# shangzhouye/stereo-visual-slam

Measured on AMD Instinct MI355X. Metric: stereo keyframes/sec (ORB+match+tri+local-BA), KITTI-00 1241x376, higher is better.
Workload: dtype u8+f64

## Files before the change

### stereo-visual-slam_amd/csrc/lm_kernels.hip

```cpp
#include "vslam_internal.h"

#include <stdlib.h>

#include <vector>

#include "se3_device.h"
#include "lm_device.h"

namespace vslam {

constexpr int kLmBlock = 512;
constexpr int kLmItemFixed = 128;
constexpr int kLmMinWaves = 2;
constexpr int kLmWaves = kLmBlock / 64;
constexpr int kMaxKf = VSLAM_MAX_KF;
constexpr int kMaxNp = 6 * kMaxKf;
constexpr int kMaxPairs = kMaxKf * (kMaxKf + 1) / 2;
constexpr int kHitsPerEdge = (kMaxKf + 1) / 2 + 1;
constexpr int kDinvLds = 1950;
constexpr int kLin = 2;
constexpr int kPoseParts = 3;
constexpr int kCntStride = 80;
constexpr int kItemSlots = (kMaxPairs + kLmWaves - 1) / kLmWaves;
constexpr int kDbgSlots = 24;
// ... 1132 lines not shown
    }
    atomicAdd(&cnt, mine);
    __syncthreads();
    if (threadIdx.x == 0 && n_inl) n_inl[b] = cnt;
}

__global__ __launch_bounds__(64) void pnp_wave_kernel(const float* __restrict__ xyz, const float* __restrict__ uv, const int32_t* __restrict__ d_n, int capacity,
                                                     double* __restrict__ d_T, int iters, double K0, double K1, double K2, double K3, double delta,
                                                     double thr2, uint8_t* __restrict__ inlier, int32_t* __restrict__ n_inl, vslam_lm_stats* __restrict__ stats) {
    const int b = blockIdx.x, lane = threadIdx.x;
    const int n = min(max(d_n[b], 0), capacity);
    const float* px = xyz + 3 * (size_t)b * capacity;
    const float2* pz = reinterpret_cast<const float2*>(uv) + (size_t)b * capacity;
    const double K[4] = {K0, K1, K2, K3};
    const CamK ck = make_camk(K);
    vslam_lm_stats* st = stats ? stats + b : nullptr;
    double T[7], Rt[12];
#pragma unroll
    for (int i = 0; i < 7; ++i) T[i] = d_T[7 * (size_t)b + i];
    expand_pose(T, Rt);
    const int slot27 = wave_slot<27>(lane);
    auto evaluate = [&](const double* R, bool lin, double (&H)[36], double (&g)[6]) -> double {
        double part = 0, acc[27];
#pragma unroll
        for (int i = 0; i < 27; ++i) acc[i] = 0;
        for (int i0 = 0; i0 < n; i0 += 128) {
            const int ia = i0 + lane, ib = i0 + 64 + lane;
            const int ja = min(ia, n - 1), jb = min(ib, n - 1);
            const double ax = px[3 * ja], ay = px[3 * ja + 1], az = px[3 * ja + 2], bx = px[3 * jb], by = px[3 * jb + 1], bz = px[3 * jb + 2];
            const float2 za = pz[ja], zb = pz[jb];
#pragma unroll
            for (int u = 0; u < 2; ++u) {
                if ((u ? ib : ia) >= n) continue;
                double x, y, ri, wgt, ex, ey, c, rho;
                cam_norm(R, u ? bx : ax, u ? by : ay, u ? bz : az, x, y, ri);
                eval_obs(ck, x, y, u ? zb : za, delta, ex, ey, c, rho, wgt);
                part += rho;
                if (lin) {
                    double A[12], wA[12];
                    jac_norm(x, y, ri, A);
                    const double l0 = wgt * ck.fx2, l1 = wgt * ck.fy2;
#pragma unroll
                    for (int i = 0; i < 6; ++i) { wA[i] = l0 * A[i]; wA[6 + i] = l1 * A[6 + i]; }
                    int idx = 0;
#pragma unroll
                    for (int r = 0; r < 6; ++r)
#pragma unroll
                        for (int cc = r; cc < 6; ++cc) { acc[idx] = a_fma_pair(wA, r, A, cc, acc[idx]); ++idx; }
#pragma unroll
                    for (int r = 0; r < 6; ++r) acc[21 + r] = a_fma2(wA, r, -ex, -ey, acc[21 + r]);
                }
            }
        }
        const double total = wave_sum(part);
        if (lin) {
            wave_reduce_scatter<27>(acc, lane);
            double v[27];
#pragma unroll
            for (int sidx = 0; sidx < 27; ++sidx) {
                const int src = __ffsll((long long)__ballot(slot27 == sidx)) - 1;
                v[sidx] = readlane_f64(acc[0], src);
            }
            int idx = 0;
#pragma unroll
            for (int r = 0; r < 6; ++r)
#pragma unroll
                for (int cc = r; cc < 6; ++cc) { H[6 * r + cc] = v[idx]; H[6 * cc + r] = v[idx]; ++idx; }
#pragma unroll
            for (int r = 0; r < 6; ++r) g[r] = v[21 + r];
        }
        return total;
    };
    double H[36], g[6], lambda = 0, ni = 2, currentChi = 0;
    int it = 0, total_trials = 0;
    for (it = 0; it < iters; ++it) {
        currentChi = evaluate(Rt, true, H, g);
        if (it == 0) {
            if (st && lane == 0) st->chi2_init = currentChi;
            double md = 0;
#pragma unroll
            for (int a = 0; a < 6; ++a) md = fmax(fabs(H[7 * a]), md);
            lambda = 1e-5 * md;
            ni = 2;
        }
        double rho_gain = 0;
        int qmax = 0;
        bool again = true;
        while (again) {
            double x[6], E[7], Tt[7], Rtt[12], Hd[36], gd[6];
            const bool ok2 = chol6_solve(H, lambda, g, x);
            if (!ok2) {
#pragma unroll
                for (int i = 0; i < 6; ++i) x[i] = 0;
            }
            se3::exp(x, E);
            se3::mul(E, T, Tt);
            expand_pose(Tt, Rtt);
            double tempChi = evaluate(Rtt, false, Hd, gd);
            if (!ok2) tempChi = 1.7976931348623157e308;
            double scale = 1e-3;
#pragma unroll
            for (int i = 0; i < 6; ++i) scale += x[i] * (lambda * x[i] + g[i]);
            rho_gain = (currentChi - tempChi) / scale;
            if (rho_gain > 0 && isfinite(tempChi)) {
                double alpha = 1. - pow(2 * rho_gain - 1, 3);
                alpha = fmin(alpha, 2. / 3.);
                lambda *= fmax(1. / 3., alpha);
                ni = 2;
                currentChi = tempChi;
#pragma unroll
                for (int i = 0; i < 7; ++i) T[i] = Tt[i];
#pragma unroll
                for (int i = 0; i < 12; ++i) Rt[i] = Rtt[i];
            } else {
                lambda *= ni;
                ni *= 2;
            }
            ++qmax;
            again = (rho_gain < 0) && qmax < 10;
        }
        total_trials += qmax;
        if (st && lane == 0 && it < VSLAM_LM_MAX_ITERS) { st->chi2_iter[it] = currentChi; st->lambda_iter[it] = lambda; st->trials_iter[it] = qmax; }
        if (qmax == 10 || rho_gain == 0) { ++it; break; }
    }
    if (st && lane == 0) { st->iterations = it; st->total_trials = total_trials; st->chi2_final = currentChi; st->lambda_final = lambda; }
    if (lane < 7) d_T[7 * (size_t)b + lane] = T[lane];
    int mine = 0;
    for (int i = lane; i < n; i += 64) {
        const size_t gi = (size_t)b * capacity + i;
        double X, Y, Z, ex, ey;
        project_err(Rt, K, (double)px[3 * i], (double)px[3 * i + 1], (double)px[3 * i + 2], uv[2 * gi], uv[2 * gi + 1], X, Y, Z, ex, ey);
        const double c = ex * ex + ey * ey;
        const bool ok = isfinite(c) && c <= thr2;
        if (inlier) inlier[gi] = ok;
        mine += ok;
    }
    for (int o = 32; o > 0; o >>= 1) mine += __shfl_xor(mine, o);
    if (lane == 0 && n_inl) n_inl[b] = mine;
}

struct PoShared {
    double H[2][kMaxKf][36], g[2][kMaxKf][6];
    double part[2][kMaxKf], spart[2][kMaxKf];
    double x[kMaxKf][6];
    int cnt[kMaxKf][kMaxKf];
    int kbeg[kMaxKf + 1];
    int flag[2];
    int cin[2][kMaxKf], cout[2][kMaxKf];
    double T[2][kMaxKf][7], R[3][kMaxKf][12];
};
template <int W, int kMinWaves>
__global__ __launch_bounds__(64 * W, kMinWaves) void pose_only_wave_kernel(LmKernelArgs ka, int iters, int update_poses) {
    static_assert(W == kMaxKf || (W >= 1 && W <= 8), "the keyframe deal takes its minimum over eight lanes");
    constexpr int kBlock = 64 * W;
    const LmWindowArgs& a = ka.a;
    __shared__ PoShared sm;
    const int w = ka.order ? ka.order[blockIdx.x] : (int)blockIdx.x, tid = threadIdx.x, lane = tid & 63;
    const int wave = __builtin_amdgcn_readfirstlane(tid >> 6);
    if (ka.status[w] != VSLAM_OK) return;
    long long* cyc = ka.dbg_cycles ? ka.dbg_cycles + kDbgSlots * (size_t)w : nullptr;
    long long t_ph = cyc ? clock64() : 0;
#define POH(i) do { if (cyc && tid == 0) { const long long t1__ = clock64(); cyc[i] += t1__ - t_ph; t_ph = t1__; } } while (0)
    const int nk = a.n_kf_w ? min(max(a.n_kf_w[w], 1), a.n_kf) : a.n_kf;
    const int lm0 = a.lm_off[w], e0 = a.edge_off[w], ne = a.edge_off[w + 1] - e0;
    const int32_t* kfi = a.kf_idx + e0;
    const int32_t* lmi = a.lm_idx + e0;
    const float2* uv2 = reinterpret_cast<const float2*>(a.uv) + e0;
    const float* xyz = a.xyz + 3 * (size_t)lm0;
    uint8_t* inl = a.lm_inlier + lm0;
    int32_t* list = a.kf_edges + e0;
    float2* uvk = reinterpret_cast<float2*>(ka.uvk) + e0;
    float4* posk = reinterpret_cast<float4*>(a.lin) + e0;
    double* chik = ka.chi2k + e0;
    const double K[4] = {a.K[0], a.K[1], a.K[2], a.K[3]};
    const CamK ck = make_camk(K);
    const double delta = a.huber_delta;
    const unsigned long long lt_mask = (1ull << lane) - 1ull;
    const int per = (((ne + W - 1) / W) + 63) & ~63;
    const int c0 = min(wave * per, ne), c1 = min(c0 + per, ne);
    {
        int cnt[kMaxKf];
#pragma unroll
        for (int k = 0; k < kMaxKf; ++k) cnt[k] = 0;
        for (int base = c0; base < c1; base += 256) {
            int kq[4], lq[4]; bool vq[4]; uint8_t iq[4];
#pragma unroll
            for (int u = 0; u < 4; ++u) { const int e = base + 64 * u + lane; vq[u] = e < c1; const int es = min(e, ne - 1); kq[u] = kfi[es]; lq[u] = lmi[es]; }
#pragma unroll
            for (int u = 0; u < 4; ++u) iq[u] = inl[lq[u]];
#pragma unroll
            for (int u = 0; u < 4; ++u) {
                const bool act = vq[u] && iq[u] != 0;
#pragma unroll
                for (int kk = 0; kk < kMaxKf; ++kk) cnt[kk] += __popcll(__ballot(act && kq[u] == kk));
            }
        }
        if (lane < kMaxKf) {
            int v = 0;
#pragma unroll
            for (int kk = 0; kk < kMaxKf; ++kk) if (lane == kk) v = cnt[kk];
            sm.cnt[wave][lane] = v;
        }
        if (tid < 2) sm.flag[tid] = 0;
    }
    __syncthreads();
    int off[kMaxKf];
    {
        int run = 0;
#pragma unroll
        for (int k = 0; k < kMaxKf; ++k) {
            int before = 0, tot = 0;
#pragma unroll
            for (int c = 0; c < W; ++c) { const int v = sm.cnt[c][k]; tot += v; if (c < wave) before += v; }
            off[k] = run + before;
            if (tid == 0) sm.kbeg[k] = run;
            run += tot;
        }
        if (tid == 0) sm.kbeg[kMaxKf] = run;
    }
    for (int base = c0; base < c1; base += 256) {
        int kq[4], lq[4], eq[4]; bool vq[4]; uint8_t iq[4]; float2 zq[4]; float Xq[4], Yq[4], Zq[4];
#pragma unroll
        for (int u = 0; u < 4; ++u) {
            const int e = base + 64 * u + lane; vq[u] = e < c1; eq[u] = e;
            const int es = min(e, ne - 1);
            kq[u] = kfi[es]; lq[u] = lmi[es]; zq[u] = uv2[es];
        }
#pragma unroll
        for (int u = 0; u < 4; ++u) { iq[u] = inl[lq[u]]; Xq[u] = xyz[3 * lq[u]]; Yq[u] = xyz[3 * lq[u] + 1]; Zq[u] = xyz[3 * lq[u] + 2]; }
#pragma unroll
        for (int u = 0; u < 4; ++u) {
            const bool act = vq[u] && iq[u] != 0;
#pragma unroll
            for (int kk = 0; kk < kMaxKf; ++kk) {
                const unsigned long long m = __ballot(act && kq[u] == kk);
                if (act && kq[u] == kk) {
                    const int pos = off[kk] + __popcll(m & lt_mask);
                    list[pos] = eq[u]; uvk[pos] = zq[u]; posk[pos] = make_float4(Xq[u], Yq[u], Zq[u], 0.f);
                }
                off[kk] += __popcll(m);
            }
        }
    }
    __syncthreads();
    POH(0);
    unsigned long long held = 0;
    int nheld = 0;
    if constexpr (W == kMaxKf) { held = (unsigned long long)wave; nheld = wave < nk ? 1 : 0; }
    else {
        const int kl = min(lane, kMaxKf - 1);
        const int mycnt = lane < nk ? sm.kbeg[kl + 1] - sm.kbeg[kl] : -1;
        int rank = 0;
        for (int j = 0; j < nk; ++j) { const int cj = sm.kbeg[j + 1] - sm.kbeg[j]; rank += (cj > mycnt || (cj == mycnt && j < lane)) ? 1 : 0; }
        int load = 0;
        for (int r = 0; r < nk; ++r) {
            const int k = __builtin_amdgcn_readfirstlane(__ffsll((long long)__ballot(lane < nk && rank == r)) - 1);
            const int cr = __shfl(mycnt, k);
            int key = lane < W ? load * 16 + lane : 0x7fffffff;
            key = min(key, __shfl_xor(key, 1)); key = min(key, __shfl_xor(key, 2)); key = min(key, __shfl_xor(key, 4));
            const int v = __builtin_amdgcn_readfirstlane(key) & 15;
            if (lane == v) load += cr;
            if (v == wave) { held |= (unsigned long long)k << (4 * nheld); ++nheld; }
        }
    }
    auto kf_at = [&](int q) -> int { return (int)((held >> (4 * q)) & 15ull); };
#pragma unroll 1
    for (int q = 0; q < nheld; ++q) {
        const int k = kf_at(q);
        double T[7], Rt[12];
#pragma unroll
        for (int i = 0; i < 7; ++i) T[i] = a.T[((size_t)w * a.n_kf + k) * 7 + i];
        expand_pose(T, Rt);
        if (lane == 0) {
#pragma unroll
            for (int i = 0; i < 7; ++i) sm.T[0][k][i] = T[i];
#pragma unroll
            for (int i = 0; i < 12; ++i) { sm.R[0][k][i] = Rt[i]; sm.R[2][k][i] = Rt[i]; }
        }
    }
    __builtin_amdgcn_wave_barrier();
    const int slot27 = wave_slot<27>(lane);
    auto evaluate = [&](const double* Rlds, bool lin, int buf, bool store_chi, int k) -> double {
        const int kb = __builtin_amdgcn_readfirstlane(sm.kbeg[k]), ke = __builtin_amdgcn_readfirstlane(sm.kbeg[k + 1]);
        double R[12];
#pragma unroll
        for (int i = 0; i < 12; ++i) R[i] = uniform_f64(Rlds[i]);
        double part = 0, acc[27];
#pragma unroll
        for (int i = 0; i < 27; ++i) acc[i] = 0;
        float4 pp[2], pn[2]; float2 zz[2], zn[2];
#pragma unroll
        for (int u = 0; u < 2; ++u) { const int j = min(kb + 64 * u + lane, max(ke - 1, 0)); pp[u] = posk[j]; zz[u] = uvk[j]; }
        for (int j0 = kb; j0 < ke; j0 += 128) {
#pragma unroll
            for (int u = 0; u < 2; ++u) { const int j = min(j0 + 128 + 64 * u + lane, ke - 1); pn[u] = posk[j]; zn[u] = uvk[j]; }
#pragma unroll
            for (int u = 0; u < 2; ++u) {
                const int j = j0 + 64 * u + lane;
                if (j >= ke) continue;
                double x, y, ri, wgt, ex, ey, c, rho;
                cam_norm(R, (double)pp[u].x, (double)pp[u].y, (double)pp[u].z, x, y, ri);
                eval_obs(ck, x, y, zz[u], delta, ex, ey, c, rho, wgt);
                part += rho;
                if (store_chi) chik[j] = c;
                if (lin) {
                    double A[12], wA[12];
                    jac_norm(x, y, ri, A);
                    const double l0 = wgt * ck.fx2, l1 = wgt * ck.fy2;
#pragma unroll
                    for (int i = 0; i < 6; ++i) { wA[i] = l0 * A[i]; wA[6 + i] = l1 * A[6 + i]; }
                    int idx = 0;
#pragma unroll
                    for (int r = 0; r < 6; ++r)
#pragma unroll
                        for (int cc = r; cc < 6; ++cc) { acc[idx] = a_fma_pair(wA, r, A, cc, acc[idx]); ++idx; }
#pragma unroll
                    for (int r = 0; r < 6; ++r) acc[21 + r] = a_fma2(wA, r, -ex, -ey, acc[21 + r]);
                }
            }
#pragma unroll
            for (int u = 0; u < 2; ++u) { pp[u] = pn[u]; zz[u] = zn[u]; }
        }
        const double total = wave_sum(part);
        if (lin) {
            wave_reduce_scatter<27>(acc, lane);
            if (slot27 >= 0 && slot27 < 21) {
                int r = 0, rem = slot27;
                while (rem >= 6 - r) { rem -= 6 - r; ++r; }
                const int cc = r + rem;
                sm.H[buf][k][6 * r + cc] = acc[0]; sm.H[buf][k][6 * cc + r] = acc[0];
            } else if (slot27 >= 21) sm.g[buf][k][slot27 - 21] = acc[0];
        }
        return total;
    };
    auto sum_kf = [&](const double* v) -> double {
        double t = 0;
        for (int k = 0; k < nk; ++k) t += v[k];
        return t;
    };
    vslam_lm_stats* st = a.stats ? a.stats + w : nullptr;
    double lambda = 0, ni = 2, currentChi = 0;
    int pc = 0;
    int cur = 0, it = 0, total_trials = 0, pb = 0, fb = 0;
    if (iters > 0) {
#pragma unroll 1
        for (int q = 0; q < nheld; ++q) {
            const int k = kf_at(q);
            const double c = evaluate(sm.R[pc][k], true, cur, false, k);
            if (lane == 0) sm.part[pb][k] = c;
        }
        __syncthreads();
        currentChi = sum_kf(sm.part[pb]);
        pb ^= 1;
        double md = 0;
        for (int k = 0; k < nk; ++k)
#pragma unroll
            for (int d = 0; d < 6; ++d) md = fmax(md, fabs(sm.H[cur][k][7 * d]));
        lambda = 1e-5 * md;
        if (st && tid == 0) st->chi2_init = currentChi;
    }
    POH(1);
    for (it = 0; it < iters; ++it) {
        double rho_gain = 0;
        int qmax = 0;
        bool again = true;
        while (again) {
            double xw[6] = {0, 0, 0, 0, 0, 0};
#pragma unroll 1
            for (int q = 0; q < nheld; ++q) {
                const int k = kf_at(q);
                double Hk[36], gk[6], x[6] = {0, 0, 0, 0, 0, 0};
#pragma unroll
                for (int i = 0; i < 36; ++i) Hk[i] = sm.H[cur][k][i];
#pragma unroll
                for (int i = 0; i < 6; ++i) gk[i] = sm.g[cur][k][i];
                if (!chol6_solve(Hk, lambda, gk, x) && lane == 0) sm.flag[fb] = 1;
                if constexpr (W == kMaxKf) {
#pragma unroll
                    for (int i = 0; i < 6; ++i) xw[i] = x[i];
                } else if (lane == 0) {
#pragma unroll
                    for (int i = 0; i < 6; ++i) sm.x[k][i] = x[i];
                }
            }
            POH(2);
            __syncthreads();
            POH(3);
            const bool ok2 = sm.flag[fb] == 0;
            if (tid == 0) sm.flag[fb ^ 1] = 0;
            fb ^= 1;
#pragma unroll 1
            for (int q = 0; q < nheld; ++q) {
                const int k = kf_at(q);
                double sc = 0;
                {
                    double x[6], E[7], Tc[7], Tt[7], Rtt[12];
#pragma unroll
                    for (int i = 0; i < 6; ++i) x[i] = !ok2 ? 0.0 : W == kMaxKf ? xw[i] : sm.x[k][i];
#pragma unroll
                    for (int i = 0; i < 6; ++i) sc += x[i] * (lambda * x[i] + sm.g[cur][k][i]);
#pragma unroll
                    for (int i = 0; i < 7; ++i) Tc[i] = sm.T[pc][k][i];
                    se3::exp(x, E);
                    se3::mul(E, Tc, Tt);
                    expand_pose(Tt, Rtt);
                    __builtin_amdgcn_wave_barrier();
                    if (lane == 0) {
#pragma unroll
                        for (int i = 0; i < 7; ++i) sm.T[pc ^ 1][k][i] = Tt[i];
#pragma unroll
                        for (int i = 0; i < 12; ++i) { sm.R[pc ^ 1][k][i] = Rtt[i]; sm.R[2][k][i] = Rtt[i]; }
                    }
                    __builtin_amdgcn_wave_barrier();
                }
                POH(4);
                const double c = evaluate(sm.R[pc ^ 1][k], true, cur ^ 1, false, k);
                POH(5);
                if (lane == 0) { sm.part[pb][k] = c; sm.spart[pb][k] = sc; }
            }
            __syncthreads();
            POH(6);
            double tempChi = sum_kf(sm.part[pb]);
            const double scale = sum_kf(sm.spart[pb]) + 1e-3;
            pb ^= 1;
            if (!ok2) tempChi = 1.7976931348623157e308;
            rho_gain = (currentChi - tempChi) / scale;
            if (rho_gain > 0 && isfinite(tempChi)) {
                double alpha = 1. - pow(2 * rho_gain - 1, 3);
                alpha = fmin(alpha, 2. / 3.);
                lambda *= fmax(1. / 3., alpha);
                ni = 2;
                currentChi = tempChi;
                pc ^= 1;
                cur ^= 1;
            } else {
                lambda *= ni;
                ni *= 2;
            }
            ++qmax;
            again = (rho_gain < 0) && qmax < 10;
        }
        total_trials += qmax;
        if (st && tid == 0 && it < VSLAM_LM_MAX_ITERS) { st->chi2_iter[it] = currentChi; st->lambda_iter[it] = lambda; st->trials_iter[it] = qmax; }
        if (qmax == 10 || rho_gain == 0) { ++it; break; }
    }
    if (st && tid == 0) { st->iterations = it; st->total_trials = total_trials; st->chi2_final = currentChi; st->lambda_final = lambda; }
    POH(7);
#pragma unroll 1
    for (int q = 0; q < nheld; ++q) { const int k = kf_at(q); evaluate(sm.R[2][k], false, 0, true, k); }
    double th = delta;
    int cb = 0;
    for (int iteration = 0; iteration < 5; ++iteration) {
#pragma unroll 1
        for (int q = 0; q < nheld; ++q) {
            const int k = kf_at(q), kb = sm.kbeg[k], ke = sm.kbeg[k + 1];
            int cin = 0, cout = 0;
            for (int j = kb + lane; j < ke; j += 64) { if (chik[j] > th) ++cout; else ++cin; }
            for (int o = 32; o > 0; o >>= 1) { cin += __shfl_xor(cin, o); cout += __shfl_xor(cout, o); }
            if (lane == 0) { sm.cin[cb][k] = cin; sm.cout[cb][k] = cout; }
        }
        __syncthreads();
        int tin = 0, tout = 0;
        for (int k = 0; k < nk; ++k) { tin += sm.cin[cb][k]; tout += sm.cout[cb][k]; }
        cb ^= 1;
        const double ratio = (double)tin / (double)(tin + tout);
        if (ratio > 0.5) break;
        th *= 2;
    }
    if (ka.want_chi2) {
        double* chi2 = a.chi2 + e0;
        for (int e = tid; e < ne; e += kBlock) if (!inl[lmi[e]]) chi2[e] = 0.0;
#pragma unroll 1
        for (int q = 0; q < nheld; ++q) {
            const int k = kf_at(q), kb = sm.kbeg[k], ke = sm.kbeg[k + 1];
            for (int j = kb + lane; j < ke; j += 64) chi2[list[j]] = chik[j];
        }
    }
    __syncthreads();
#pragma unroll 1
    for (int q = 0; q < nheld; ++q) {
        const int k = kf_at(q), kb = sm.kbeg[k], ke = sm.kbeg[k + 1];
        for (int j = kb + lane; j < ke; j += 64) {
            const int e = list[j];
            if (e == ne - 1 || lmi[e + 1] != lmi[e]) inl[lmi[e]] = !(chik[j] > th);
        }
        if (update_poses && lane < 7) a.T[((size_t)w * a.n_kf + k) * 7 + lane] = sm.T[pc][k][lane];
    }
    if (tid == 0 && a.chi2_thr) a.chi2_thr[w] = th;
    POH(8);
#undef POH
}

static int carve_lm(LmScratch& s, LmKernelArgs& ka, size_t total_lm, size_t total_edge, int n_windows, bool with_lm, hipStream_t stream) {
    int32_t* defer;
    if (int rc = carve(s.buf, stream, [&](Layout& L) {
            ka.a.P = L.take<double>(total_lm * 3);
            ka.a.Ptrial = L.take<double>(total_lm * 3);
            ka.a.Hll = L.take<double>(total_lm * 6);
            ka.a.bl = L.take<double>(total_lm * 3);
            ka.a.Dinv = L.take<double>(total_lm * 6);
            ka.a.lin = L.take<double>(total_edge * kLin);
            ka.a.lm_ptr = L.take<int32_t>(total_lm + n_windows + 1);
            ka.a.kf_ptr = L.take<int32_t>((size_t)n_windows * (kMaxKf + 1));
            ka.a.kf_edges = L.take<int32_t>(total_edge);
            ka.a.pair_ptr = L.take<int32_t>((size_t)n_windows * (kMaxPairs + 1));
            ka.a.pair_hits = L.take<int32_t>(with_lm ? total_edge * kHitsPerEdge * 2 : 64);
            ka.act = L.take<uint8_t>(total_lm);
            ka.kf_pos = L.take<int32_t>(total_edge);
            ka.status = L.take<int32_t>(n_windows);
            double* chi2 = L.take<double>(total_edge);
            if (!ka.a.chi2) ka.a.chi2 = chi2;
            ka.chi2k = L.take<double>(total_edge);
            ka.uvk = L.take<float>(total_edge * 2);
            ka.slot_uv = L.take<float>(with_lm ? total_lm * kLmSlots * 2 : 64);
            ka.slot_kf = L.take<uint8_t>(with_lm ? total_lm * kLmSlots : 256);
            ka.lcnt = L.take<uint8_t>(total_lm);
            ka.order = L.take<int32_t>(n_windows);
            ka.passes = L.take<int32_t>(n_windows);
            defer = L.take<int32_t>(n_windows);
        })) return rc;
    s.status = ka.status; s.status_n = n_windows; s.passes = ka.passes; s.defer = defer;
    return VSLAM_OK;
}

__global__ void lm_fill_kernel(int32_t* __restrict__ p, int n, int v) { const int i = blockIdx.x * blockDim.x + threadIdx.x; if (i < n) p[i] = v; }
constexpr int kOrderCap = 4096;
__global__ __launch_bounds__(1024) void lm_order_kernel(const int32_t* __restrict__ edge_off, int n, int32_t* __restrict__ order) {
    __shared__ unsigned long long key[kOrderCap];
    int np2 = 1;
    while (np2 < n) np2 <<= 1;
    for (int i = threadIdx.x; i < np2; i += 1024)
        key[i] = i < n ? ((unsigned long long)(0xFFFFFFFFu - (unsigned)max(edge_off[i + 1] - edge_off[i], 0)) << 32) | (unsigned)i : ~0ull;
    for (int k = 2; k <= np2; k <<= 1)
        for (int j = k >> 1; j > 0; j >>= 1) {
            __syncthreads();
            for (int t = threadIdx.x; t < np2 / 2; t += 1024) {
                const int lo = ((t / j) * 2 * j) + (t % j), hi = lo + j;
                const bool up = (lo & k) == 0;
                const unsigned long long x = key[lo], y = key[hi];
                if ((x > y) == up) { key[lo] = y; key[hi] = x; }
            }
        }
    __syncthreads();
    for (int i = threadIdx.x; i < n; i += 1024) order[i] = (int32_t)(key[i] & 0xFFFFFFFFu);
}

int launch_lm_windows(const LmWindowArgs& a, int schedule, int mode, int iters, int update_poses, int update_lms, LmScratch* scratch,
                      hipStream_t stream) {
    const size_t total_lm = a.total_lm, total_edge = a.total_edge;
    if (a.n_windows <= 0) return VSLAM_OK;
    if (a.n_kf <= 0 || a.n_kf > kMaxKf) { set_error("n_kf %d out of range (1..%d)", a.n_kf, kMaxKf); return VSLAM_ERR_ARG; }
    LmKernelArgs ka;
    memset(&ka, 0, sizeof(ka));
    ka.a = a;
    ka.want_chi2 = a.chi2 != nullptr;
    ka.dinv_lds = kDinvLds;
    const size_t dyn_lds = (size_t)kDinvLds * 6 * sizeof(double);
    if (!scratch->lds_opt_in) {
        VS_HIP(hipFuncSetAttribute(reinterpret_cast<const void*>(&lm_window_kernel<false>), hipFuncAttributeMaxDynamicSharedMemorySize, (int)dyn_lds));
        VS_HIP(hipFuncSetAttribute(reinterpret_cast<const void*>(&lm_window_kernel<false, true>), hipFuncAttributeMaxDynamicSharedMemorySize, (int)dyn_lds));
        scratch->lds_opt_in = true;
    }
    if (getenv("VSLAM_LM_PROFILE")) {
        const size_t cyc_need = sizeof(long long) * kDbgSlots * a.n_windows;
        if (int rc = scratch->cyc.reserve(cyc_need, stream)) return rc;
        VS_HIP(hipMemsetAsync(scratch->cyc.p, 0, cyc_need, stream));
        ka.dbg_cycles = (long long*)scratch->cyc.p;
    }
    int rc = carve_lm(*scratch, ka, total_lm, total_edge, a.n_windows, true, stream);
    if (rc) return rc;
    const bool adaptive = !(scratch->tune && scratch->tune->ba_adaptive == 0);
    const bool resident_on = (schedule || mode == 0) && !(scratch->tune && scratch->tune->ba_resident == 0);
// ... 162 lines not shown
```

### stereo-visual-slam_amd/csrc/vslam_internal.h

```cpp
#pragma once
#include <hip/hip_runtime.h>
#include <stdint.h>
#include <stdio.h>
#include <string.h>

#include "../../include/vslam_hip.h"

namespace vslam {

void set_error(const char* fmt, ...);

#define VS_HIP(call)                                                                              \
    do {                                                                                          \
        hipError_t e__ = (call);                                                                  \
        if (e__ != hipSuccess) {                                                                  \
            ::vslam::set_error("%s:%d %s -> %s", __FILE__, __LINE__, #call, hipGetErrorString(e__)); \
            return VSLAM_ERR_HIP;                                                                 \
        }                                                                                         \
    } while (0)

struct Prof;
Prof* prof_current();
void prof_set_current(Prof* p);
void prof_begin(hipStream_t s, const char* name, int launches);
// ... 30 lines not shown
    layout(m);
    if (int rc = buf.reserve(m.off, stream)) return rc;
    a.base = buf.p; a.off = 0;
    layout(a);
    if (a.off > buf.bytes) { set_error("%s layout uses %zu bytes of %zu reserved", buf.name, a.off, buf.bytes); return VSLAM_ERR_CAPACITY; }
    return VSLAM_OK;
}
template <typename F>
int carve(DevBuf& buf, hipStream_t stream, F&& layout) { Layout a; return carve(buf, stream, a, layout); }

constexpr int kWave = 64;
constexpr int kNLevels = VSLAM_ORB_NLEVELS;
constexpr int kEdge = 31;
constexpr int kMaxRows = 4096;

struct OrbLevel {
    int w, h;
    float scale;
    int nfeat;
    int pyr_off;
    int corner_cap;
    int corner_off;
    int tiles_x, tiles_y, tile_off;
    int tab_off;
};

struct OrbPlan {
    OrbLevel lv[kNLevels];
    int w, h;
    int pyr_bytes;
    int corner_total;
    int total_tiles;
    int sel_cap;
    int blur_off[kNLevels];
    int blur_bytes;
};

struct Ctx;

struct OrbTables {
    int* d_xofs;
    short* d_ialpha;
    int* d_yofs;
    short* d_ibeta;
    int x_off[kNLevels], y_off[kNLevels];
    int* d_tile_dx;
    int* d_tile_dy;
    int tdx_off[kNLevels], tdy_off[kNLevels];
    size_t bytes;
};

void orb_debug_enable();
void orb_debug_dump(hipStream_t stream);
int orb_plan_init(OrbPlan* plan, int w, int h, int nfeatures, int kp_capacity);
int orb_tables_init(const OrbPlan* plan, OrbTables* t);
void orb_tables_free(OrbTables* t);

struct OrbBuffers {
    uint8_t* d_pyr;
    uint32_t* d_corners;
    int32_t* d_corner_cnt;
    vslam_keypoint* d_sel;
    int32_t* d_sel_cnt;
    int32_t* d_status;
    vslam_keypoint* d_det;
    uint8_t* d_blur;
    float2* d_cs;
    int32_t* d_order;
    double* d_rad;
    int32_t* d_anms_path;
};

int launch_orb_pyramid(const OrbPlan& plan, const OrbTables& tab, const uint8_t* d_imgs, size_t img_bytes, int pitch,
                       int B, uint8_t* d_pyr, hipStream_t stream);
int launch_orb_pyrblur(const OrbPlan& plan, const OrbTables& tab, const uint8_t* d_imgs, size_t img_bytes, int pitch, int B, uint8_t* d_pyr,
                       uint8_t* d_blur, int fast_thr, uint32_t* d_corners, int32_t* d_corner_cnt, int32_t* d_status, hipStream_t stream);
int launch_orb_fast(const OrbPlan& plan, const uint8_t* d_imgs, size_t img_bytes, int pitch, int B, const uint8_t* d_pyr,
                    int fast_thr, uint32_t* d_corners, int32_t* d_corner_cnt, int32_t* d_status, hipStream_t stream);
int launch_orb_select(const OrbPlan& plan, const uint8_t* d_imgs, size_t img_bytes, int pitch, int B, const uint8_t* d_pyr,
                      const uint32_t* d_corners, const int32_t* d_corner_cnt, vslam_keypoint* d_sel, int32_t* d_sel_cnt,
                      int32_t* d_status, hipStream_t stream);
int launch_orb_anms(const OrbPlan& plan, int B, const vslam_keypoint* d_sel, const int32_t* d_sel_cnt, int sel_cap,
                    int anms_num, int regroup, vslam_keypoint* d_kps, float2* d_cs, int32_t* d_order, int kp_capacity, int32_t* d_count, int32_t* d_status,
                    double* d_rad, int anms_cap, int32_t* d_path, hipStream_t stream);
int launch_anms_flat(int B, const vslam_keypoint* d_in, const int32_t* d_nin, int in_capacity, int anms_num, int regroup,
                     int img_w, int img_h, vslam_keypoint* d_kps, float2* d_cs, int32_t* d_order, int kp_capacity, int32_t* d_count, int32_t* d_status,
                     double* d_rad, int anms_cap, int32_t* d_path, hipStream_t stream);
int launch_orb_blur(const OrbPlan& plan, const uint8_t* d_imgs, size_t img_bytes, int pitch, int B, const uint8_t* d_pyr, uint8_t* d_blur,
                    hipStream_t stream);
int launch_orb_orient(const OrbPlan& plan, const uint8_t* d_imgs, size_t img_bytes, int pitch, int B, const uint8_t* d_pyr, vslam_keypoint* d_kps,
                      float2* d_cs, const int32_t* d_order, int kp_capacity, const int32_t* d_count, hipStream_t stream);
int launch_orb_describe(const OrbPlan& plan, const uint8_t* d_imgs, size_t img_bytes, int pitch, int B, const uint8_t* d_pyr,
                        const uint8_t* d_blur, const vslam_keypoint* d_kps, const float2* d_cs, const int32_t* d_order, int kp_capacity, const int32_t* d_count,
                        uint8_t* d_desc, hipStream_t stream);

struct MatchBuffers {
    uint32_t* d_train_best;
};
int launch_match(const uint8_t* d_q, size_t q_stride, const int32_t* d_nq, const uint8_t* d_t, size_t t_stride,
                 const int32_t* d_nt, const double* d_gap, int gate, double ratio, double gap_thr, int B, int max_rows,
                 uint32_t* d_train_best, vslam_dmatch* d_out, int out_capacity, int32_t* d_nout, hipStream_t stream,
                 const int32_t* d_qsel = nullptr, int sel_cap = 0, const int32_t* d_nqsel = nullptr, const int32_t* d_qitem = nullptr, int n_qitems = 0);

struct CamParams { double fx, fy, cx, cy, b, dmin, dmax, drel, row_tol; };
int launch_find3d_disparity(const vslam_keypoint* d_kps, int n, const float* d_disp, int w, int h, int dstride,
                            const double* d_T, CamParams cam, float* d_xyz, uint8_t* d_valid, uint8_t* d_rel, hipStream_t stream);
int launch_find3d_disparity_batch(const vslam_keypoint* d_kps, const int32_t* d_n, int kp_capacity, int B, const float* d_disp, int w, int h,
                                  const double* d_T, CamParams cam, float* d_xyz, uint8_t* d_valid, uint8_t* d_rel, hipStream_t stream);
int launch_triangulate(const float* d_uvL, const float* d_uvR, const int32_t* d_n, int capacity, int B, const double* d_T,
                       CamParams cam, float* d_xyz, uint8_t* d_valid, uint8_t* d_rel, hipStream_t stream);
int launch_build_pnp_inputs(const vslam_dmatch* d_m, const int32_t* d_nm, int match_capacity, const vslam_dmatch* d_lr,
                            const int32_t* d_nlr, int lr_capacity, const float* d_xyz_lr, const uint8_t* d_valid_lr,
                            const vslam_keypoint* d_kpsT, int kp_capacity, int B, int32_t* d_kp2lr, float* d_xyz_out, float* d_uv_out,
                            int32_t* d_nout, int out_capacity, hipStream_t stream, const int32_t* d_seg_start = nullptr);
int launch_gather_uv(const vslam_keypoint* d_kpsQ, const vslam_keypoint* d_kpsT, int kp_capacity, const vslam_dmatch* d_m,
                     const int32_t* d_nm, int match_capacity, int B, float* d_uvQ, float* d_uvT, hipStream_t stream);

int launch_hbm_copy_probe(const void* src, void* dst, size_t bytes, int variant, hipStream_t stream);
int hbm_copy_probe_variants();
const char* hbm_copy_probe_name(int variant);

struct LmWindowArgs {
    int n_windows, n_kf;
    const int32_t* n_kf_w;
    const int32_t* lm_off;
    const int32_t* edge_off;
    double* T;
    float* xyz;
    const uint8_t* reliable;
    uint8_t* lm_inlier;
    const int32_t* kf_idx;
    const int32_t* lm_idx;
    const float* uv;
    double* chi2;
    vslam_lm_stats* stats;
    double* P;
    double* Ptrial;
    double* Hll;
    double* bl;
    double* Dinv;
    double* lin;
    int32_t* lm_ptr;
    int32_t* kf_ptr;
    int32_t* kf_edges;
    int32_t* pair_ptr;
    int32_t* pair_hits;
    int32_t hit_capacity_per_edge;
    double K[4];
    double huber_delta;
    double* chi2_thr;
    size_t total_lm, total_edge;
};
constexpr int kPoseOnlyNarrowWaves = 4;
struct Tuning {
    int orb_fuse_min = -1;
    int anms_cap = -1;
    int sgbm_fuse_min = -1;
    int sgbm_fwd_min = -1;
    int sgbm_fw_rows = -1;
    int pose_only_window = -1;
    int pose_only_waves = -1;
    int pnp_window = -1;
    int ba_lanes = -1;
    int ba_resident = -1;
    int track_rule = -1;
    int rectify_form = -1;
    int ba_adaptive = -1;
};
constexpr int kSgbmTicketPools = 8;
constexpr int kSgbmErrorWord = kSgbmTicketPools;
int launch_sgbm(const Tuning& tune, const vslam_sgbm_params& sp, const uint8_t* d_left, const uint8_t* d_right, size_t img_bytes, int pitch, int w, int h, int B,
                float* d_disp_f32, int16_t* d_disp_i16, int16_t* d_disp_raw, DevBuf& scratch, hipStream_t stream);

struct LmScratch {
    DevBuf buf, cyc;
    int32_t* status = nullptr; int status_n = 0;
    int32_t* passes = nullptr;
    const Tuning* tune = nullptr;
    bool lds_opt_in = false;
    bool rs_opt_in = false;
    int rs_dyn_bytes = -1, rs_full_bytes = 0, rs_cu_count = 0;
    int32_t* defer = nullptr;
    bool defer_valid = false;
    explicit LmScratch(size_t* acct) : buf("LM scratch", acct), cyc("LM clock buffer", acct) {}
};
struct RsLaunch {
    LmWindowArgs a;
    void* uv_s; int32_t* epos; double* tab; double* xin; double* Pbak; double* Dc; double* blc;
    int32_t* status; int32_t* passes; int32_t* defer; const int32_t* order; long long* dbg;
    int dyn_bytes, full_bytes, cu_count;
    int schedule, adaptive, iters, update_poses, update_lms, dense_to_general;
    int want_chi2;
    int lanes;
    bool opt_in_done;
};
void rs_query_device(int device, LmScratch& s);
int launch_ba_resident(const RsLaunch& L, hipStream_t stream);
int launch_lm_windows(const LmWindowArgs& a, int schedule, int mode, int iters, int update_poses, int update_lms, LmScratch* scratch,
                      hipStream_t stream);
size_t lm_hits_per_edge();
int lm_fetch_status(const LmScratch* scratch, int n_windows, int32_t* h_status, hipStream_t stream);
int lm_fetch_passes(const LmScratch* scratch, int n_windows, int32_t* h_passes, hipStream_t stream);
int lm_fetch_deferred(const LmScratch* scratch, int n_windows, int32_t* h_defer, hipStream_t stream);

struct PnpArgs {
    const float* xyz; const float* uv; const int32_t* n; int capacity; int B;
    double* T; int iters; double K[4]; double huber_delta; double reproj_thr;
    uint8_t* inlier; int32_t* n_inliers; vslam_lm_stats* stats;
    int n_hint;
};
int launch_pnp(const PnpArgs& a, LmScratch* scratch, hipStream_t stream);
int launch_edge_jacobians(int n, const float* d_xyz, const float* d_uv, const double* d_T, const double K[4], double delta, double* d_err, double* d_Jp, double* d_Jl,
                          double* d_chi2, double* d_hw, hipStream_t stream);
size_t pnp_epnp_ws_bytes(int H);
int launch_pnp_epnp(const float* d_hx, const float* d_hu, int H, const double K[4], double* d_Rt, double* d_T, int32_t* d_ok, uint8_t* ws, hipStream_t stream);
int launch_pnp_count_inliers(const float* d_xyz, const float* d_uv, int n, const double* d_Rt, const int32_t* d_ok, int hyp0, int n_hyp, const double K[4],
                             double reproj_thr, int32_t* d_counts, uint8_t* d_mask, hipStream_t stream);

int launch_pnp_ransac_batch(const float* d_xyz, const float* d_uv, const int32_t* d_n, int capacity, int B, int H, const double K[4], double reproj_err,
                            double confidence, DevBuf& scratch, double* d_T, uint8_t* d_inlier, int32_t* d_n_inl, int32_t* d_iters, hipStream_t stream);
struct KfPolicy { int policy; double near_dist; int32_t* kf_frame; int32_t* evicted; bool gate = false; const int32_t* num_inliers = nullptr; int32_t* frame_state = nullptr;
                  const double* G = nullptr; const int32_t* in_of_match = nullptr; const int32_t* state_in = nullptr;
                  bool recover = false; const int32_t* pred_table = nullptr; };
struct SegView { const int32_t* start = nullptr; const int32_t* first = nullptr; const int32_t* qitem = nullptr; int n_seg = 0; };
int launch_seg_expand(int n_frames, int n_seg, const int32_t* d_first, int32_t* d_start, int32_t* d_qitem, hipStream_t stream);
int launch_build_windows(const vslam_tracks_in& in, int n_kf, int lm_capacity, int edge_capacity, const double K4[4], double reproj_thr, int track_rule, DevBuf& scratch,
                         int32_t* d_lm_off, int32_t* d_edge_off, int32_t* d_n_kf, double* d_T, float* d_xyz_out, uint8_t* d_rel_out, uint8_t* d_inl_out,
                         int32_t* d_kf_out, int32_t* d_lm_out, float* d_uv_out, int32_t* d_status, const KfPolicy& kp, hipStream_t stream, const SegView& seg);
int launch_chain_poses(int n_frames, const double* d_T_rel, double* d_G, hipStream_t stream, const SegView& seg);
int launch_gate_states(int n_frames, const double* d_T, int absolute, const int32_t* d_num_inliers, int32_t* d_state, hipStream_t stream, const SegView& seg);
int launch_frame_pairs(int n_frames, const int32_t* d_state, int32_t* d_pred, double* d_gap, hipStream_t stream, const SegView& seg);
int launch_gate_states_pairs(int n_frames, const double* d_G, const int32_t* d_pred, const int32_t* d_num_inliers, int32_t* d_state, DevBuf& scratch,
                             hipStream_t stream, const SegView& seg);
struct MapRecover { const int32_t* d_pred_prev; int32_t* d_pred; double* d_gap; };
struct MapRequery { const uint8_t* d_desc; size_t desc_stride; int32_t* d_feat; int32_t* d_nfeat; vslam_dmatch* d_f2f_out; int32_t* d_nf2f_out;
                    double ratio, gap_thr; uint32_t* d_train_best; };
int launch_map_pnp_inputs(const vslam_tracks_in& in, const double* d_G, const int32_t* d_in_of_match_prev, const int32_t* d_state, const double K4[4],
                          double reproj_thr, int track_rule, DevBuf& scratch, float* d_xyz_out, float* d_uv_out, int32_t* d_n_out, int32_t* d_in_of_match,
                          int out_capacity, int32_t* d_status, hipStream_t stream, const SegView& seg, const MapRequery* rq = nullptr, const MapRecover* rv = nullptr);

constexpr int kRectifyGroup = 8;
void rectify_rotation_error(const double R[9], double* ortho_err, double* det);
void rectify_build_map(const vslam_rectify_cam& cam, int dst_w, int dst_h, int16_t* xy, uint16_t* frac);
int rectify_map_pitch(int dst_w);
void rectify_pack_map(const int16_t* xy, const uint16_t* frac, int dst_w, int dst_h, int src_w, int src_h, uint2* out);
int rectify_tiles_x(int dst_w);
void rectify_tile_boxes(const uint2* packed, int dst_w, int dst_h, int4* tiles);
struct RectifyLaunch { const uint2* map[2]; const int4* tiles[2]; const uint8_t* src[2]; uint8_t* dst[2]; int w, h, B, src_pitch, dst_pitch, form;
                       size_t src_img_bytes, dst_img_bytes; };
int launch_rectify(const RectifyLaunch& L, hipStream_t stream);
struct RectifyState { uint2* d_map[2]; int4* d_tiles[2]; int src_w[2], src_h[2]; };

struct Ctx {
    vslam_params p;
    int device;
    hipStream_t stream;
    bool own_stream;
    size_t dev_bytes;
    OrbPlan plan;
    OrbTables tab;
    OrbBuffers orb;
    MatchBuffers match;
    DevBuf stage{"staging", &dev_bytes, (size_t)1 << 20};
    uint8_t* h_pinned; size_t pinned_bytes;
    DevBuf sgbm{"SGBM scratch", &dev_bytes};
    bool sgbm_unchecked;
    DevBuf ransac{"RANSAC scratch", &dev_bytes};
    DevBuf track{"track scratch", &dev_bytes};
    LmScratch lm{&dev_bytes};
    Tuning tune;
    Prof* prof;
    RectifyState rect;
    DevBuf segbuf{"segment table", &dev_bytes};
    SegView seg;
    int seg_frames;
    bool orb_ok;
};

}
```

Measured before the change: 68210.

## Cache setup edge codes in registers and split per-keyframe pose math across lane groups

In the pose-only LM kernel, the first 24 rows of edges per wave are loaded once during the counting pass. Their landmark indices and packed 4-bit keyframe codes are kept in registers so the scatter pass does not reload kfi, lmi and the inlier flags. The per-keyframe pose setup, Cholesky solve and SE3 update now run in 8-lane groups, so several held keyframes are handled at once instead of one at a time with lane 0 writing. The update step is also separated from the evaluation loop. This costs extra register pressure and duplicated loop code, and it relies on kMaxKf < 15.

```diff
diff --git a/stereo-visual-slam_amd/csrc/lm_kernels.hip b/stereo-visual-slam_amd/csrc/lm_kernels.hip
--- a/stereo-visual-slam_amd/csrc/lm_kernels.hip
+++ b/stereo-visual-slam_amd/csrc/lm_kernels.hip
@@ -1308,6 +1308,7 @@
 template <int W, int kMinWaves>
 __global__ __launch_bounds__(64 * W, kMinWaves) void pose_only_wave_kernel(LmKernelArgs ka, int iters, int update_poses) {
     static_assert(W == kMaxKf || (W >= 1 && W <= 8), "the keyframe deal takes its minimum over eight lanes");
+    static_assert(kMaxKf < 15 && kPoSetupRows == 8 && kPoSetupKeep % kPoSetupRows == 0, "a kept row is four bits of a dword, 15 = not active");
     constexpr int kBlock = 64 * W;
     const LmWindowArgs& a = ka.a;
     __shared__ PoShared sm;
@@ -1334,11 +1335,38 @@
     const unsigned long long lt_mask = (1ull << lane) - 1ull;
     const int per = (((ne + W - 1) / W) + 63) & ~63;
     const int c0 = min(wave * per, ne), c1 = min(c0 + per, ne);
+    constexpr int kKeep = W == kMaxKf ? 0 : kPoSetupKeep, kTrips = kKeep / kPoSetupRows;
+    int lmk[kKeep + 1];
+    unsigned code[kTrips + 1];
+    const int cr = min(c0 + 64 * kKeep, c1);
     {
         int cnt[kMaxKf];
 #pragma unroll
         for (int k = 0; k < kMaxKf; ++k) cnt[k] = 0;
-        for (int base = c0; base < c1; base += 256) {
+#pragma unroll
+        for (int t = 0; t < kTrips; ++t) {
+            const int base = c0 + 64 * kPoSetupRows * t;
+            code[t] = ~0u;
+#pragma unroll
+            for (int u = 0; u < kPoSetupRows; ++u) lmk[kPoSetupRows * t + u] = 0;
+            if (base < c1) {
+                int kq[kPoSetupRows]; uint8_t iq[kPoSetupRows];
+#pragma unroll
+                for (int u = 0; u < kPoSetupRows; ++u) { const int es = min(base + 64 * u + lane, ne - 1); kq[u] = kfi[es]; lmk[kPoSetupRows * t + u] = lmi[es]; }
+#pragma unroll
+                for (int u = 0; u < kPoSetupRows; ++u) iq[u] = inl[lmk[kPoSetupRows * t + u]];
+                unsigned c = 0;
+#pragma unroll
+                for (int u = 0; u < kPoSetupRows; ++u) {
+                    const int cd = (base + 64 * u + lane < c1 && iq[u] != 0) ? kq[u] : 15;
+                    c |= (unsigned)cd << (4 * u);
+#pragma unroll
+                    for (int kk = 0; kk < kMaxKf; ++kk) cnt[kk] += __popcll(__ballot(cd == kk));
+                }
+                code[t] = c;
+            }
+        }
+        for (int base = cr; base < c1; base += 256) {
             int kq[4], lq[4]; bool vq[4]; uint8_t iq[4];
 #pragma unroll
             for (int u = 0; u < 4; ++u) { const int e = base + 64 * u + lane; vq[u] = e < c1; const int es = min(e, ne - 1); kq[u] = kfi[es]; lq[u] = lmi[es]; }
@@ -1374,7 +1402,32 @@
         }
         if (tid == 0) sm.kbeg[kMaxKf] = run;
     }
-    for (int base = c0; base < c1; base += 256) {
+#pragma unroll
+    for (int t = 0; t < kTrips; ++t) {
+        const int base = c0 + 64 * kPoSetupRows * t;
+        if (base < c1) {
+            float2 zq[kPoSetupRows]; float Xq[kPoSetupRows], Yq[kPoSetupRows], Zq[kPoSetupRows];
+#pragma unroll
+            for (int u = 0; u < kPoSetupRows; ++u) {
+                const int l = lmk[kPoSetupRows * t + u];
+                zq[u] = uv2[min(base + 64 * u + lane, ne - 1)]; Xq[u] = xyz[3 * l]; Yq[u] = xyz[3 * l + 1]; Zq[u] = xyz[3 * l + 2];
+            }
+#pragma unroll
+            for (int u = 0; u < kPoSetupRows; ++u) {
+                const int cd = (int)((code[t] >> (4 * u)) & 15u);
+#pragma unroll
+                for (int kk = 0; kk < kMaxKf; ++kk) {
+                    const unsigned long long m = __ballot(cd == kk);
+                    if (cd == kk) {
+                        const int pos = off[kk] + __popcll(m & lt_mask);
+                        list[pos] = base + 64 * u + lane; uvk[pos] = zq[u]; posk[pos] = make_float4(Xq[u], Yq[u], Zq[u], 0.f);
+                    }
+                    off[kk] += __popcll(m);
+                }
+            }
+        }
+    }
+    for (int base = cr; base < c1; base += 256) {
         int kq[4], lq[4], eq[4]; bool vq[4]; uint8_t iq[4]; float2 zq[4]; float Xq[4], Yq[4], Zq[4];
 #pragma unroll
         for (int u = 0; u < 4; ++u) {
@@ -1420,14 +1473,18 @@
         }
     }
     auto kf_at = [&](int q) -> int { return (int)((held >> (4 * q)) & 15ull); };
+    constexpr int kGroupLanes = W == kMaxKf ? 64 : kPoGroupLanes, kGroups = 64 / kGroupLanes;
+    const int grp = lane / kGroupLanes;
+    const bool glead = lane % kGroupLanes == 0;
 #pragma unroll 1
-    for (int q = 0; q < nheld; ++q) {
-        const int k = kf_at(q);
+    for (int q0 = 0; q0 < nheld; q0 += kGroups) {
+        const bool mine = q0 + grp < nheld;
+        const int k = kf_at(mine ? q0 + grp : 0);
         double T[7], Rt[12];
 #pragma unroll
         for (int i = 0; i < 7; ++i) T[i] = a.T[((size_t)w * a.n_kf + k) * 7 + i];
         expand_pose(T, Rt);
-        if (lane == 0) {
+        if (mine && glead) {
 #pragma unroll
             for (int i = 0; i < 7; ++i) sm.T[0][k][i] = T[i];
 #pragma unroll
@@ -1523,18 +1580,19 @@
         while (again) {
             double xw[6] = {0, 0, 0, 0, 0, 0};
 #pragma unroll 1
-            for (int q = 0; q < nheld; ++q) {
-                const int k = kf_at(q);
+            for (int q0 = 0; q0 < nheld; q0 += kGroups) {
+                const bool mine = q0 + grp < nheld;
+                const int k = kf_at(mine ? q0 + grp : 0);
                 double Hk[36], gk[6], x[6] = {0, 0, 0, 0, 0, 0};
 #pragma unroll
                 for (int i = 0; i < 36; ++i) Hk[i] = sm.H[cur][k][i];
 #pragma unroll
                 for (int i = 0; i < 6; ++i) gk[i] = sm.g[cur][k][i];
-                if (!chol6_solve(Hk, lambda, gk, x) && lane == 0) sm.flag[fb] = 1;
+                if (!chol6_solve(Hk, lambda, gk, x) && mine && glead) sm.flag[fb] = 1;
                 if constexpr (W == kMaxKf) {
 #pragma unroll
                     for (int i = 0; i < 6; ++i) xw[i] = x[i];
-                } else if (lane == 0) {
+                } else if (mine && glead) {
 #pragma unroll
                     for (int i = 0; i < 6; ++i) sm.x[k][i] = x[i];
                 }
@@ -1546,34 +1604,38 @@
             if (tid == 0) sm.flag[fb ^ 1] = 0;
             fb ^= 1;
 #pragma unroll 1
+            for (int q0 = 0; q0 < nheld; q0 += kGroups) {
+                const bool mine = q0 + grp < nheld;
+                const int k = kf_at(mine ? q0 + grp : 0);
+                double sc = 0;
+                double x[6], E[7], Tc[7], Tt[7], Rtt[12];
+#pragma unroll
+                for (int i = 0; i < 6; ++i) x[i] = !ok2 ? 0.0 : W == kMaxKf ? xw[i] : sm.x[k][i];
+#pragma unroll
+                for (int i = 0; i < 6; ++i) sc += x[i] * (lambda * x[i] + sm.g[cur][k][i]);
+#pragma unroll
+                for (int i = 0; i < 7; ++i) Tc[i] = sm.T[pc][k][i];
+                se3::exp(x, E);
+                se3::mul(E, Tc, Tt);
+                expand_pose(Tt, Rtt);
+                __builtin_amdgcn_wave_barrier();
+                if (mine && glead) {
+#pragma unroll
+                    for (int i = 0; i < 7; ++i) sm.T[pc ^ 1][k][i] = Tt[i];
+#pragma unroll
+                    for (int i = 0; i < 12; ++i) { sm.R[pc ^ 1][k][i] = Rtt[i]; sm.R[2][k][i] = Rtt[i]; }
+                    sm.spart[pb][k] = sc;
+                }
+                __builtin_amdgcn_wave_barrier();
+            }
+            POH(4);
+#pragma unroll 1
             for (int q = 0; q < nheld; ++q) {
                 const int k = kf_at(q);
-                double sc = 0;
-                {
-                    double x[6], E[7], Tc[7], Tt[7], Rtt[12];
-#pragma unroll
-                    for (int i = 0; i < 6; ++i) x[i] = !ok2 ? 0.0 : W == kMaxKf ? xw[i] : sm.x[k][i];
-#pragma unroll
-                    for (int i = 0; i < 6; ++i) sc += x[i] * (lambda * x[i] + sm.g[cur][k][i]);
-#pragma unroll
-                    for (int i = 0; i < 7; ++i) Tc[i] = sm.T[pc][k][i];
-                    se3::exp(x, E);
-                    se3::mul(E, Tc, Tt);
-                    expand_pose(Tt, Rtt);
-                    __builtin_amdgcn_wave_barrier();
-                    if (lane == 0) {
-#pragma unroll
-                        for (int i = 0; i < 7; ++i) sm.T[pc ^ 1][k][i] = Tt[i];
-#pragma unroll
-                        for (int i = 0; i < 12; ++i) { sm.R[pc ^ 1][k][i] = Rtt[i]; sm.R[2][k][i] = Rtt[i]; }
-                    }
-                    __builtin_amdgcn_wave_barrier();
-                }
-                POH(4);
                 const double c = evaluate(sm.R[pc ^ 1][k], true, cur ^ 1, false, k);
-                POH(5);
-                if (lane == 0) { sm.part[pb][k] = c; sm.spart[pb][k] = sc; }
-            }
+                if (lane == 0) sm.part[pb][k] = c;
+            }
+            POH(5);
             __syncthreads();
             POH(6);
             double tempChi = sum_kf(sm.part[pb]);
diff --git a/stereo-visual-slam_amd/csrc/vslam_internal.h b/stereo-visual-slam_amd/csrc/vslam_internal.h
--- a/stereo-visual-slam_amd/csrc/vslam_internal.h
+++ b/stereo-visual-slam_amd/csrc/vslam_internal.h
@@ -206,6 +206,9 @@
     size_t total_lm, total_edge;
 };
 constexpr int kPoseOnlyNarrowWaves = 4;
+constexpr int kPoSetupRows = 8;
+constexpr int kPoSetupKeep = 24;
+constexpr int kPoGroupLanes = 8;
 struct Tuning {
     int orb_fuse_min = -1;
     int anms_cap = -1;
```

After: 68510 (median of 6 runs). Within noise of the previous version (+0.4%).
